# smolGura/fish-tts

Measured on AMD Instinct MI355X. Metric: semantic tokens/sec, higher is better.
Workload: dtype bf16; 1 GPU; openaudio-s1-mini shapes (BASELINE configs[1]): batch=1 per GPU, 48-token prompt, 215 frames (10 s), top-p sampling, hipGraph-captured frame step, + DAC codec decode; prompt_len=48, parallelism=replica x1, frame_engine=3

## Files before the change

fish-tts_amd/csrc/ar_kernels.h:

```cpp
#pragma once
#include "common.h"

namespace ft {

enum { PRO_NONE = 0, PRO_RMSNORM = 1 };
enum { EPI_STORE = 0, EPI_RESID = 1, EPI_SWIGLU = 2 };

__device__ __host__ __forceinline__ size_t xo_index(int m, int k, int ldm) { return ((size_t)(k >> 3) * ldm + m) * 8 + (k & 7); }

struct GemvP {
    const void* W;
    const void* bias;
    const float* x;
    int ldx;
    const void* gain;
    float eps;
    float* out;
    int ldo;
    const float* resid;
    int ldr;
    int N, K;
    int pro, epi;
    int nt;
};
// ... 1396 lines not shown
#pragma unroll
        for (int c = 1; c <= 4; ++c) {
            const unsigned long long bal = __ballot(mine >= c);
            below += __popcll(bal & lower);
            wtot += __popcll(bal);
        }
        if (lane == 0) wcnt[wave] = wtot;
        __syncthreads();
        int rank = below;
        for (int w = 0; w < wave; ++w) rank += wcnt[w];
        bool keep[4];
        float et[4], z2 = 0.f;
#pragma unroll
        for (int e = 0; e < 4; ++e) {
            keep[e] = (i0 + e) < V && (all_kept || key[e] > kstar || (mem[e] && rank < nk));
            rank += mem[e] ? 1 : 0;
            et[e] = keep[e] ? expf(rb<ROUND>(l[e] / Tc) - Mt) : 0.f;
            z2 += et[e];
        }
        const float Z2 = red.sum(z2);
        const float* qrow = nullptr;
        if (p.noise && nfv < p.noise_rows) qrow = p.noise + (size_t)nfv * p.noise_row_len + p.noise_off;
        float q4[4];
        draw_noise4(p, ctl, qrow, i0, nfv, m, V, q4);
        ArgMax best{-1.f, 0x7fffffff};
#pragma unroll
        for (int e = 0; e < 4; ++e) {
            if (i0 + e < V) {
                const float prob = keep[e] ? rb<ROUND>(et[e] / Z2) : 0.f;
                best = better(best, ArgMax{rb<ROUND>(prob / rb<ROUND>(q4[e])), i0 + e});
            }
        }
        winner = block_best(best).i;
    }
    __syncthreads();
    finish_draw<WT>(p, m, winner, nfv);
}

struct SampCut {
    unsigned kstar;
    int nk;
    int all_kept;
    int argmax;
    float Lmax, Mt, Z2, Tc;
};

struct SampBigP {
    SampP s;
    SampCut* cut;
    int* chunk_cnt;
    float* part_score;
    int* part_idx;
    int nchunk;
};

__device__ __forceinline__ float key16_value(unsigned k16) {
    const uint32_t k = k16 << 16;
    const uint32_t u = (k & 0x80000000u) ? (k & 0x7fffffffu) : ~(k | 0xffffu);
    return __uint_as_float(u);
}

constexpr int SAMP_TH_THREADS = 1024;
constexpr int SAMP_TH_ROW = 33;
constexpr int SAMP_TH_OVF = 8;
constexpr size_t SAMP_TH_LDS = (size_t)SAMP_TH_THREADS * SAMP_TH_ROW * 4;

struct SampThShared {
    float red[16];
    int redi[16];
    float wsum[16];
    int wact[16];
    int AL[1024];
    unsigned ovf_key[SAMP_TH_OVF];
    unsigned ovf_cnt[SAMP_TH_OVF];
    int ovf_n;
    SampCut cut_s;
};

__device__ __forceinline__ void samp_cut_from_image(const SampBigP& b, const int m, const uint32_t* cimg, SampThShared& sh,
                                                    const bool has, const int kmax_t) {
    const SampP& p = b.s;
    const int tid = threadIdx.x, lane = tid & 63, wave = tid >> 6;
    const RowCtl ctl = p.ctl[m];
    float* red = sh.red;
    int* redi = sh.redi;
    float* wsum = sh.wsum;
    int* wact = sh.wact;
    int* AL = sh.AL;
    unsigned* ovf_key = sh.ovf_key;
    unsigned* ovf_cnt = sh.ovf_cnt;
    int& ovf_n = sh.ovf_n;
    SampCut& cut_s = sh.cut_s;
    const unsigned long long hb = __ballot(has);
    if (lane == 0) wact[wave] = __popcll(hb);
    __syncthreads();
    int abase = 0, n_active = 0;
    for (int w = 0; w < 16; ++w) { if (w < wave) abase += wact[w]; n_active += wact[w]; }
    if (has) AL[abase + __popcll(hb & ((1ull << lane) - 1ull))] = tid;
    ArgMax km = block_argmax(ArgMax{(float)kmax_t, tid}, red, redi);
    const unsigned kmax = (unsigned)(int)km.v;
    const float Lmax = key16_value(kmax);
    const int n_items = n_active * 64;
    const int ipt = (n_items + 1023) / 1024;
    const int i0 = tid * ipt, i1 = min(i0 + ipt, n_items);
    auto item_count = [&](int i, unsigned& k) -> float {
        const int g = AL[i >> 6], j = i & 63;
        k = 64u * g + j;
        const uint32_t w = cimg[g * SAMP_TH_ROW + (j >> 1)];
        unsigned c = (j & 1) ? (w >> 16) : (w & 0xffffu);
        if (c == 65535u)
            for (int q = 0; q < ovf_n && q < SAMP_TH_OVF; ++q) if (ovf_key[q] == k) c = ovf_cnt[q];
        return (float)c;
    };
    float z = 0.f;
    for (int i = i0; i < i1; ++i) {
        unsigned k;
        const float c = item_count(i, k);
        if (c > 0.f) z = fmaf(c, expf(key16_value(k) - Lmax), z);
    }
    const float Z = block_sum(z, red);
    const float tp = round_bf16(ctl.top_p);
    auto removed = [&](float cum) { return round_bf16(cum) > tp; };
    auto prob = [&](unsigned k16) { return round_bf16(expf(key16_value(k16) - Lmax) / Z); };
    float mt = 0.f;
    for (int i = i0; i < i1; ++i) {
        unsigned k;
        const float c = item_count(i, k);
        if (c > 0.f) mt = fmaf(c, prob(k), mt);
    }
    float suf = mt;
#pragma unroll
    for (int o = 1; o < 64; o <<= 1) {
        const float t = __shfl_down(suf, o, 64);
        if (lane + o < 64) suf += t;
    }
    __syncthreads();
    if (lane == 0) wsum[wave] = suf;
    __syncthreads();
    float above = suf - mt;
    for (int w = wave + 1; w < 16; ++w) above += wsum[w];
    int found = -1;
    unsigned f_key = 0;
    float f_above = 0.f, f_cnt = 0.f;
    float run = above;
    for (int i = i1 - 1; i >= i0; --i) {
        unsigned k;
        const float c = item_count(i, k);
        if (c > 0.f) {
            const float nxt = fmaf(c, prob(k), run);
            if (found < 0 && removed(nxt)) { found = i; f_key = k; f_above = run; f_cnt = c; }
            run = nxt;
        }
    }
    ArgMax who = block_argmax(ArgMax{found >= 0 ? (float)tid : -1.f, tid}, red, redi);
    if (tid == 0) { cut_s.all_kept = who.v < 0.f ? 1 : 0; cut_s.kstar = 0; cut_s.nk = 0; }
    __syncthreads();
    if (who.v >= 0.f && tid == (int)who.v) {
        const float pk = prob(f_key);
        int lo_n = 0, hi_n = (int)f_cnt;
        while (lo_n < hi_n) {
            const int mid = (lo_n + hi_n + 1) >> 1;
            if (removed(fmaf((float)mid, pk, f_above))) hi_n = mid - 1; else lo_n = mid;
        }
        if (f_key == kmax && lo_n < 1) lo_n = 1;
        cut_s.kstar = f_key;
        cut_s.nk = lo_n;
    }
    __syncthreads();
    const unsigned kstar = cut_s.kstar;
    const int nk = cut_s.nk, all_kept = cut_s.all_kept;
    const float Tc = fmaxf(ctl.temperature, 1e-5f);
    const float Mt = round_bf16(Lmax / Tc);
    float z2 = 0.f;
    for (int i = i0; i < i1; ++i) {
        unsigned k;
        const float c = item_count(i, k);
        if (c > 0.f) {
            float n = 0.f;
            if (all_kept || k > kstar) n = c;
            else if (k == kstar) n = (float)nk;
            if (n > 0.f) z2 = fmaf(n, expf(round_bf16(key16_value(k) / Tc) - Mt), z2);
        }
    }
    const float Z2 = block_sum(z2, red);
    if (tid == 0) {
        SampCut o;
        o.kstar = kstar; o.nk = nk; o.all_kept = all_kept; o.argmax = 0;
        o.Lmax = Lmax; o.Mt = Mt; o.Z2 = Z2; o.Tc = Tc;
        b.cut[m] = o;
    }
}

static __global__ __launch_bounds__(1024) void samp_cut_kernel(SampBigP b) {
    extern __shared__ __attribute__((aligned(16))) uint32_t cimg[];
    __shared__ SampThShared sh;
    __shared__ int pen_id[32];
    __shared__ float pen_val[32];
    const SampP& p = b.s;
    const int m = blockIdx.x, tid = threadIdx.x;
    float* L = p.logits + (size_t)m * p.ldl;
    const int V = p.V;
    const RowCtl ctl = p.ctl[m];
    const int nfv = p.nf[m];
    const int R = p.ncb + 1;
    const int* seq = p.seq + (size_t)m * R * p.cap;
    for (int i = tid; i < SAMP_TH_THREADS * SAMP_TH_ROW; i += 1024) cimg[i] = 0u;
    if (tid == 0) sh.ovf_n = 0;
    const int npen = nfv > 0 ? (p.cb == 0 ? R : 16) : 0;
    auto count1 = [&](float v) {
        const unsigned k = order_key(v) >> 16;
        atomicAdd(&cimg[(k >> 6) * SAMP_TH_ROW + ((k & 63u) >> 1)], (k & 1u) ? 0x10000u : 1u);
    };
    {
        if (nfv > 0) {
            const int it = nfv - 1;
            const int ws = it < 16 ? 0 : it - 16;
            if (tid < npen) {
                const int id = p.cb == 0 ? seq[(size_t)tid * p.cap + ws + 1] : seq[(size_t)(p.cb + 1) * p.cap + ws + 1 + tid];
                pen_id[tid] = -1;
                if (id >= 0 && id < V) {
                    const float sv = L[id];
                    pen_id[tid] = id;
                    pen_val[tid] = sv < 0.f ? round_bf16(sv * ctl.rep) : round_bf16(sv / ctl.rep);
                }
            }
            __syncthreads();
            if (tid < npen && pen_id[tid] >= 0) L[pen_id[tid]] = pen_val[tid];
        }
        if (p.cb == 0 && ctl.ban_eos && tid == 0 && p.im_end < V) L[p.im_end] = -INFINITY;
        __syncthreads();
        const int V16 = ((reinterpret_cast<uintptr_t>(L) & 15) == 0) ? (V / 16384) * 16384 : 0;
        float4 fa[4], fb[4];
        auto ld16 = [&](float4 (&f)[4], int base) {
#pragma unroll
            for (int u = 0; u < 4; ++u) f[u] = *reinterpret_cast<const float4*>(L + base + u * 4096 + tid * 4);
        };
        auto cnt16 = [&](const float4 (&f)[4]) {
#pragma unroll
            for (int u = 0; u < 4; ++u) { count1(f[u].x); count1(f[u].y); count1(f[u].z); count1(f[u].w); }
        };
        if (V16 > 0) ld16(fa, 0);
        for (int base = 0; base < V16; base += 32768) {
            if (base + 16384 < V16) ld16(fb, base + 16384);
            cnt16(fa);
            if (base + 32768 < V16) ld16(fa, base + 32768);
            if (base + 16384 < V16) cnt16(fb);
        }
        for (int base = V16; base < V; base += 4096) {
            float f[4];
#pragma unroll
            for (int u = 0; u < 4; ++u) { const int i = base + u * 1024 + tid; f[u] = i < V ? L[i] : 0.f; }
#pragma unroll
            for (int u = 0; u < 4; ++u) if (base + u * 1024 + tid < V) count1(f[u]);
        }
    }
    __syncthreads();
    const uint32_t* row = cimg + tid * SAMP_TH_ROW;
    int kmax_t = -1;
    unsigned tot = 0;
#pragma unroll 8
    for (int j = 0; j < 32; ++j) {
        const uint32_t w = row[j];
        const unsigned c0 = w & 0xffffu, c1 = w >> 16;
        if (c0) kmax_t = 64 * tid + 2 * j;
        if (c1) kmax_t = 64 * tid + 2 * j + 1;
        tot += c0 + c1;
    }
    const int total = (int)block_sum((float)tot, sh.red);
    if (total != V) {
        __shared__ unsigned exc_key[SAMP_TH_OVF];
        __shared__ unsigned exc_cnt[SAMP_TH_OVF];
        for (int i = tid; i < SAMP_TH_THREADS * SAMP_TH_ROW; i += 1024) cimg[i] = 0u;
        if (tid < SAMP_TH_OVF) { exc_key[tid] = 0xffffffffu; exc_cnt[tid] = 0u; }
        __syncthreads();
        for (int i = tid; i < V; i += 1024) {
            const unsigned k = order_key(L[i]) >> 16;
            uint32_t* d = &cimg[(k >> 6) * SAMP_TH_ROW + ((k & 63u) >> 1)];
            const unsigned shft = (k & 1u) * 16u;
            for (;;) {
                const uint32_t old = *reinterpret_cast<volatile uint32_t*>(d);
                if (((old >> shft) & 0xffffu) == 65535u) {
                    for (int q = 0; q < SAMP_TH_OVF; ++q) {
                        const unsigned prev = atomicCAS(&exc_key[q], 0xffffffffu, k);
                        if (prev == 0xffffffffu || prev == k) { atomicAdd(&exc_cnt[q], 1u); break; }
                    }
                    break;
                }
                if (atomicCAS(d, old, old + (1u << shft)) == old) break;
            }
        }
        __syncthreads();
        if (tid == 0) {
            int n = 0;
            for (int q = 0; q < SAMP_TH_OVF; ++q)
                if (exc_key[q] != 0xffffffffu) { sh.ovf_key[n] = exc_key[q]; sh.ovf_cnt[n] = 65535u + exc_cnt[q]; ++n; }
            sh.ovf_n = n;
        }
        kmax_t = -1;
        tot = 0;
        for (int j = 0; j < 32; ++j) {
            const uint32_t w = row[j];
            if (w & 0xffffu) kmax_t = 64 * tid + 2 * j;
            if (w >> 16) kmax_t = 64 * tid + 2 * j + 1;
            tot += (w & 0xffffu) + (w >> 16);
        }
        __syncthreads();
    }
    samp_cut_from_image(b, m, cimg, sh, tot != 0u, kmax_t);
}

static __global__ __launch_bounds__(256) void samp_count_kernel(SampBigP b) {
    __shared__ float red[4];
    const SampP& p = b.s;
    const int m = blockIdx.y, tid = threadIdx.x;
    const int c0 = blockIdx.x * 1024;
    const float* L = p.logits + (size_t)m * p.ldl;
    const SampCut cut = b.cut[m];
    float c = 0.f;
#pragma unroll
    for (int e = 0; e < 4; ++e) {
        const int i = c0 + 4 * tid + e;
        if (i < p.V && (order_key(L[i]) >> 16) == cut.kstar) c += 1.f;
    }
    c = wave_sum(c);
    if ((tid & 63) == 0) red[tid >> 6] = c;
    __syncthreads();
    if (tid == 0) b.chunk_cnt[(size_t)m * b.nchunk + blockIdx.x] = (int)(red[0] + red[1] + red[2] + red[3]);
}

static __global__ __launch_bounds__(256) void samp_race_kernel(SampBigP b) {
    __shared__ float red[4];
    __shared__ int redi[4];
    __shared__ int wcnt[4];
    const SampP& p = b.s;
    const int m = blockIdx.y, tid = threadIdx.x, lane = tid & 63, wave = tid >> 6;
    const int c0 = blockIdx.x * 1024;
    const float* L = p.logits + (size_t)m * p.ldl;
    const int V = p.V;
    const RowCtl ctl = p.ctl[m];
    const int nfv = p.nf[m];
    const SampCut cut = b.cut[m];
    float basef = 0.f;
    for (int i = tid; i < (int)blockIdx.x; i += 256) basef += (float)b.chunk_cnt[(size_t)m * b.nchunk + i];
    basef = wave_sum(basef);
    if (lane == 0) red[wave] = basef;
    __syncthreads();
    const int base = (int)(red[0] + red[1] + red[2] + red[3]);
    __syncthreads();
    float l[4];
    bool member[4];
    int mine = 0;
#pragma unroll
    for (int e = 0; e < 4; ++e) {
        const int i = c0 + 4 * tid + e;
        l[e] = i < V ? L[i] : -INFINITY;
        member[e] = i < V && !cut.all_kept && (order_key(l[e]) >> 16) == cut.kstar;
        mine += member[e] ? 1 : 0;
    }
    int incl = mine;
#pragma unroll
    for (int o = 1; o < 64; o <<= 1) {
// ... 53 lines not shown
```

fish-tts_amd/csrc/engine.h:

```cpp
#pragma once
#include <hip/hip_runtime.h>

#include <map>
#include <string>
#include <vector>

#include "../../include/fishtts_hip.h"
#include "../../include/fishtts_hip_test.h"
#include "common.h"

namespace ft {
struct RowCtl;
struct SampCut;
struct EngLayer;
}

struct FtTensor {
    void* p = nullptr;
    std::vector<int64_t> shape;
    int dtype = FT_BF16;
    int64_t numel() const {
        int64_t n = 1;
        for (auto s : shape) n *= s;
        return n;
// ... 11 lines not shown

struct ft_ctx {
    ft_ar_config c{};
    bool has_ar = false;
    ft_codec_config cc{};
    bool has_codec = false;
    int device = 0;
    hipStream_t stream = nullptr;
    std::string err;
    bool finalized = false;

    std::map<std::string, FtTensor> expected;
    size_t esz = 2;

    void *emb = nullptr, *cb_emb = nullptr, *norm = nullptr, *head = nullptr, *fproj_w = nullptr,
         *fproj_b = nullptr, *fast_emb = nullptr, *fast_norm = nullptr, *fast_out = nullptr;
    float *rope = nullptr, *frope = nullptr;
    std::vector<FtLayer> layers, flayers;

    float *x = nullptr, *qkv = nullptr, *y = nullptr, *g = nullptr, *logits = nullptr, *hid = nullptr,
          *femb = nullptr, *xf = nullptr, *qkvf = nullptr, *gf = nullptr, *flog = nullptr, *part_o = nullptr,
          *part_ml = nullptr;
    int n_slots = 0, nsplit = 1, cap = 0, fastV = 0, y_ld = 0;
    int nsplit_max = 1;
    bool nsplit_fixed = false;
    float *pf_x = nullptr, *pf_qkv = nullptr, *pf_y = nullptr;
    ft::bf16_t *pf_xn = nullptr, *pf_ybf = nullptr, *pf_g = nullptr, *pf_qbf = nullptr;
    int4* pf_seqs = nullptr;
    int2* pf_rows = nullptr;
    ft::bf16_t *xo_x = nullptr, *xo_xf = nullptr, *xo_femb = nullptr, *xo_y = nullptr, *xo_g = nullptr;
    ft::bf16_t* wide_qkv0_tab = nullptr;
    int xo_ldm = 0;
    int xo_pair = 0;
    bool no_attn_wide = false;
    bool no_head_stream = false;
    bool no_pair = false;
    int wide_min = 5;
    bool wide_ok = false;
    bool prefill_v0 = false;
    int prefill_gemm_mode = 2;
    size_t cache_m_stride = 0, fcache_m_stride = 0;

    int *d_pos = nullptr, *d_tok = nullptr, *d_tokn = nullptr, *d_seq = nullptr, *d_nf = nullptr,
        *d_done = nullptr, *d_prompt = nullptr;
    ft::RowCtl* d_ctl = nullptr;
    int *h_pin = nullptr;
    float* noise = nullptr;
    long noise_rows = 0, noise_row_len = 0;

    ft::SampCut* samp_cut = nullptr;
    int* samp_chunk_cnt = nullptr;
    float* samp_part_score = nullptr;
    int* samp_part_idx = nullptr;

    bool eng_on = false;
    bool eng_fast_on = false;
    int eng_nb = 0;
    ft::EngLayer *eng_layers = nullptr, *eng_flayers = nullptr;
    unsigned *eng_gx = nullptr, *eng_gqkv = nullptr, *eng_gy = nullptr, *eng_gxb = nullptr, *eng_gg = nullptr;
    unsigned long long* eng_gpart = nullptr;
    unsigned* eng_fast_g = nullptr;
    unsigned* eng_ctl = nullptr;
    size_t eng_lds_slow = 0, eng_lds_fast = 0, eng_fast_words = 0, eng_pool_words = 0;
    bool eng_relay = true;
    void* eng_qkv0_tab = nullptr;
    bool eng_pair = false;
    bool xl_shape = false;
    bool eng_xl = false;
    std::string path_str;
    const void* eng_slow_fn = nullptr;
    const void* eng_fast_fn = nullptr;
    size_t eng_pool_bytes = 0, eng_gpart_bytes = 0, eng_fast_bytes = 0;
    bool eng_suspended = false;
    int eng_strikes = 0, eng_last_where = 0;
    bool eng_owner = false;
    std::string eng_why;

    std::map<int, hipGraphExec_t> graphs;
    std::map<int, int> graph_nodes;

    bool prof = false, prof_count_only = false;
    std::vector<hipEvent_t> prof_ev;
    int64_t prof_bytes = 0, prof_launches = 0;

    CodecState* codec = nullptr;
};

ft_status ft_fail(ft_ctx* ctx, ft_status code, const std::string& msg);
#define FT_HIP(ctx, call)                                                                         \
    do {                                                                                          \
        hipError_t e_ = (call);                                                                   \
        if (e_ != hipSuccess)                                                                     \
            return ft_fail(ctx, FT_ERR_HIP, std::string(#call) + ": " + hipGetErrorString(e_));  \
    } while (0)

ft_status codec_create(ft_ctx* ctx);
void codec_destroy(ft_ctx* ctx);
void codec_expected(ft_ctx* ctx);
void ft_expect(ft_ctx* ctx, const std::string& name, std::vector<int64_t> shape, int dtype);
ft_status codec_finalize(ft_ctx* ctx);
```

fish-tts_amd/csrc/engine.hip:

```cpp
#include "engine.h"
#include "ar_kernels.h"
#include "frame_engine.h"
#include "wide_kernels.h"
#include "codec_kernels.h"

#include <math.h>

#include <algorithm>
#include <mutex>
#include <stdio.h>
#include <stdlib.h>
#include <string.h>

using namespace ft;

static std::string g_create_err;
static void eng_release(ft_ctx* ctx);

ft_status ft_fail(ft_ctx* ctx, ft_status code, const std::string& msg) {
    if (ctx) ctx->err = msg; else g_create_err = msg;
    return code;
}

template <typename S, typename D>
// ... 138 lines not shown
        FT_TRY(dmalloc(ctx, (char**)&l.vc, M * ctx->cache_m_stride * ctx->esz));
    }
    for (auto& l : ctx->flayers) {
        FT_TRY(dmalloc(ctx, (char**)&l.kc, M * ctx->fcache_m_stride * ctx->esz));
        FT_TRY(dmalloc(ctx, (char**)&l.vc, M * ctx->fcache_m_stride * ctx->esz));
    }
    const size_t R = c.num_codebooks + 1;
    FT_TRY(dmalloc(ctx, &ctx->d_pos, M));
    FT_TRY(dmalloc(ctx, &ctx->d_tok, M * R));
    FT_TRY(dmalloc(ctx, &ctx->d_tokn, M * R));
    FT_TRY(dmalloc(ctx, &ctx->d_seq, M * R * ctx->cap));
    FT_TRY(dmalloc(ctx, &ctx->d_nf, M));
    FT_TRY(dmalloc(ctx, &ctx->d_done, M));
    FT_TRY(dmalloc(ctx, &ctx->d_prompt, R * (size_t)c.max_seq_len));
    FT_TRY(dmalloc(ctx, &ctx->d_ctl, M));
    ctx->prefill_gemm_mode = getenv("FT_PREFILL_GEMM") ? atoi(getenv("FT_PREFILL_GEMM")) : 2;
    ctx->prefill_v0 = getenv("FT_PREFILL_V0") != nullptr || c.dtype != FT_BF16 || c.dim % 32 || (c.n_head * c.head_dim) % 32 ||
                      c.intermediate_size % 32;
    if (!ctx->prefill_v0) {
        const size_t S = c.max_seq_len;
        FT_TRY(dmalloc(ctx, &ctx->pf_x, S * c.dim));
        FT_TRY(dmalloc(ctx, &ctx->pf_qkv, S * qkvN));
        FT_TRY(dmalloc(ctx, &ctx->pf_y, S * c.n_head * c.head_dim));
        FT_TRY(dmalloc(ctx, &ctx->pf_xn, S * c.dim));
        FT_TRY(dmalloc(ctx, &ctx->pf_ybf, S * c.n_head * c.head_dim));
        FT_TRY(dmalloc(ctx, &ctx->pf_g, S * c.intermediate_size));
        FT_TRY(dmalloc(ctx, &ctx->pf_qbf, S * c.n_head * c.head_dim));
        FT_TRY(dmalloc(ctx, &ctx->pf_seqs, M));
        FT_TRY(dmalloc(ctx, &ctx->pf_rows, S));
        const int HD = c.n_head * c.head_dim, HDf = c.fast_n_head * c.fast_head_dim;
        ctx->wide_ok = !getenv("FT_NO_WIDE") && !c.fast_attention_qkv_bias && !c.fast_attention_o_bias && c.fast_dim == c.dim &&
                       wide_k_ok(c.dim) && wide_k_ok(HD) && wide_k_ok(c.intermediate_size) && wide_k_ok(HDf) && wide_k_ok(c.fast_intermediate_size) &&
                       qkvN % 32 == 0 && fqkvN % 32 == 0 && c.intermediate_size % 16 == 0 && c.fast_intermediate_size % 16 == 0 &&
                       c.dim % 16 == 0 && c.vocab_size % 32 == 0 && ctx->fastV % 16 == 0;
        if (ctx->wide_ok) {
            ctx->xo_pair = (int)((M + 15) / 16 * 16);
            ctx->no_pair = getenv("FT_NO_PAIR") != nullptr;
            ctx->no_attn_wide = getenv("FT_NO_ATTN_WIDE") != nullptr;
            ctx->no_head_stream = getenv("FT_NO_HEAD_STREAM") != nullptr;
            ctx->xo_ldm = 2 * ctx->xo_pair;
            const size_t P = ctx->xo_ldm;
            FT_TRY(dmalloc(ctx, &ctx->xo_x, P * c.dim));
            FT_TRY(dmalloc(ctx, &ctx->xo_xf, P * c.fast_dim));
            FT_TRY(dmalloc(ctx, &ctx->xo_femb, P * c.fast_dim));
            FT_TRY(dmalloc(ctx, &ctx->xo_y, P * (size_t)std::max(HD, HDf)));
            FT_TRY(dmalloc(ctx, &ctx->xo_g, P * (size_t)std::max(c.intermediate_size, c.fast_intermediate_size)));
        }
    }
    const size_t nchunk = ((size_t)c.vocab_size + 1023) / 1024;
    FT_TRY(dmalloc(ctx, &ctx->samp_cut, M));
    FT_TRY(dmalloc(ctx, &ctx->samp_chunk_cnt, M * nchunk));
    FT_TRY(dmalloc(ctx, &ctx->samp_part_score, M * nchunk));
    FT_TRY(dmalloc(ctx, &ctx->samp_part_idx, M * nchunk));
    FT_HIP(ctx, hipHostMalloc((void**)&ctx->h_pin, (3 * M + 8) * sizeof(int), hipHostMallocDefault));
    return FT_OK;
}

extern "C" ft_status ft_create(const ft_ar_config* ar, const ft_codec_config* codec, int32_t device, ft_ctx** out) {
    if (!out || (!ar && !codec)) return ft_fail(nullptr, FT_ERR_ARG, "ft_create: need a config and an out pointer");
    int ndev = 0;
    if (hipGetDeviceCount(&ndev) != hipSuccess || ndev == 0)
        return ft_fail(nullptr, FT_ERR_HIP, "ft_create: no HIP device visible (the MI355X path has no CPU fallback)");
    if (device < 0 || device >= ndev) return ft_fail(nullptr, FT_ERR_ARG, "ft_create: bad device index");
    ft_ctx* ctx = new ft_ctx();
    ctx->device = device;
    ft_status st = FT_OK;
    do {
        if (hipSetDevice(device) != hipSuccess) { st = ft_fail(ctx, FT_ERR_HIP, "hipSetDevice failed"); break; }
        if (hipStreamCreateWithFlags(&ctx->stream, hipStreamNonBlocking) != hipSuccess) {
            st = ft_fail(ctx, FT_ERR_HIP, "hipStreamCreate failed"); break;
        }
        if (ar) {
            ctx->c = *ar;
            ctx->has_ar = true;
            if ((st = ar_validate(ctx)) != FT_OK) break;
            if ((st = ar_alloc(ctx)) != FT_OK) break;
            ar_expected(ctx);
        }
        if (codec) {
            ctx->cc = *codec;
            ctx->has_codec = true;
            if ((st = codec_create(ctx)) != FT_OK) break;
            codec_expected(ctx);
        }
    } while (0);
    if (st != FT_OK) {
        g_create_err = ctx->err;
        ft_destroy(ctx);
        return st;
    }
    *out = ctx;
    return FT_OK;
}

extern "C" void ft_destroy(ft_ctx* ctx) {
    if (!ctx) return;
    hipSetDevice(ctx->device);
    if (ctx->stream) hipStreamSynchronize(ctx->stream);
    for (auto& kv : ctx->graphs) hipGraphExecDestroy(kv.second);
    for (auto& kv : ctx->expected) if (kv.second.p) hipFree(kv.second.p);
    for (auto& l : ctx->layers) { hipFree(l.kc); hipFree(l.vc); if (l.w13) hipFree(l.w13); }
    for (auto& l : ctx->flayers) { hipFree(l.kc); hipFree(l.vc); if (l.w13) hipFree(l.w13); }
    float* bufs[] = {ctx->x, ctx->qkv, ctx->y, ctx->g, ctx->logits, ctx->femb, ctx->xf, ctx->qkvf, ctx->gf,
                     ctx->flog, ctx->part_o, ctx->part_ml, ctx->noise};
    for (float* b : bufs) if (b) hipFree(b);
    if (ctx->hid && ctx->hid != ctx->x) hipFree(ctx->hid);
    int* ibufs[] = {ctx->d_pos, ctx->d_tok, ctx->d_tokn, ctx->d_seq, ctx->d_nf, ctx->d_done, ctx->d_prompt};
    for (int* b : ibufs) if (b) hipFree(b);
    if (ctx->d_ctl) hipFree(ctx->d_ctl);
    if (ctx->wide_qkv0_tab) hipFree(ctx->wide_qkv0_tab);
    { void* pf[] = {ctx->pf_x, ctx->pf_qkv, ctx->pf_y, ctx->pf_xn, ctx->pf_ybf, ctx->pf_g, ctx->xo_x, ctx->xo_xf, ctx->xo_femb, ctx->xo_y, ctx->xo_g, ctx->pf_qbf}; for (void* q : pf) if (q) hipFree(q); }
    for (auto& l : ctx->layers) { if (l.bqkv_f32) hipFree(l.bqkv_f32); if (l.bo_f32) hipFree(l.bo_f32); }
    if (ctx->samp_cut) hipFree(ctx->samp_cut);
    if (ctx->samp_chunk_cnt) hipFree(ctx->samp_chunk_cnt);
    if (ctx->samp_part_score) hipFree(ctx->samp_part_score);
    if (ctx->samp_part_idx) hipFree(ctx->samp_part_idx);
    eng_release(ctx);
    if (ctx->h_pin) hipHostFree(ctx->h_pin);
    for (auto e : ctx->prof_ev) hipEventDestroy(e);
    codec_destroy(ctx);
    if (ctx->stream) hipStreamDestroy(ctx->stream);
    delete ctx;
}

extern "C" const char* ft_last_error(const ft_ctx* ctx) { return ctx ? ctx->err.c_str() : g_create_err.c_str(); }

extern "C" ft_status ft_sync(ft_ctx* ctx) {
    if (!ctx) return FT_ERR_ARG;
    FT_HIP(ctx, hipSetDevice(ctx->device));
    FT_HIP(ctx, hipStreamSynchronize(ctx->stream));
    return FT_OK;
}

extern "C" ft_status ft_load_weight(ft_ctx* ctx, const char* name, const void* src, int32_t src_dtype,
                                    const int64_t* shape, int32_t ndim) {
    if (!ctx || !name || !src || !shape) return ft_fail(ctx, FT_ERR_ARG, "ft_load_weight: null argument");
    if (ctx->finalized) return ft_fail(ctx, FT_ERR_STATE, "ft_load_weight: weights already finalized");
    auto it = ctx->expected.find(name);
    if (it == ctx->expected.end()) return ft_fail(ctx, FT_ERR_ARG, std::string("unknown weight name: ") + name);
    FtTensor& t = it->second;
    if ((int)t.shape.size() != ndim) return ft_fail(ctx, FT_ERR_ARG, std::string("rank mismatch for ") + name);
    for (int i = 0; i < ndim; ++i)
        if (t.shape[i] != shape[i]) {
            char buf[256];
            snprintf(buf, sizeof buf, "shape mismatch for %s: dim %d is %lld, expected %lld", name, i,
                     (long long)shape[i], (long long)t.shape[i]);
            return ft_fail(ctx, FT_ERR_ARG, buf);
        }
    if (src_dtype != FT_F32 && src_dtype != FT_BF16 && src_dtype != FT_F16)
        return ft_fail(ctx, FT_ERR_ARG, "src_dtype must be FT_F32, FT_BF16 or FT_F16");
    FT_HIP(ctx, hipSetDevice(ctx->device));
    const int64_t n = t.numel();
    const size_t ssz = src_dtype == FT_F32 ? 4 : 2, dsz = t.dtype == FT_F32 ? 4 : 2;
    if (!t.p) FT_HIP(ctx, hipMalloc(&t.p, (size_t)n * dsz + 64));
    if (src_dtype == t.dtype) {
        FT_HIP(ctx, hipMemcpy(t.p, src, (size_t)n * dsz, hipMemcpyDefault));
        return FT_OK;
    }
    void* stage = nullptr;
    FT_HIP(ctx, hipMalloc(&stage, (size_t)n * ssz));
    hipError_t e = hipMemcpy(stage, src, (size_t)n * ssz, hipMemcpyDefault);
    if (e == hipSuccess) {
        const int blocks = (int)((n + 255) / 256 < 4096 ? (n + 255) / 256 : 4096);
        auto to = [&](auto* sp) {
            if (t.dtype == FT_F32) convert_kernel<<<blocks, 256, 0, ctx->stream>>>(sp, (float*)t.p, n);
            else if (t.dtype == FT_BF16) convert_kernel<<<blocks, 256, 0, ctx->stream>>>(sp, (bf16_t*)t.p, n);
            else convert_kernel<<<blocks, 256, 0, ctx->stream>>>(sp, (f16_t*)t.p, n);
        };
        if (src_dtype == FT_F32) to((const float*)stage);
// ... 727 lines not shown
                                                                             ctx->xo_x + (size_t)L.m0 * 8, ctx->xo_ldm);
            L.chk();
        }
        if constexpr (ROUND == RND_BF16)
            wide_gemm(L, ctx->xo_x + (size_t)L.m0 * 8, ctx->head, nullptr, c.vocab_size, c.dim, ctx->norm, WEPI_STORE,
                      ctx->logits + (size_t)L.m0 * c.vocab_size, c.vocab_size, nullptr, nullptr, 0, true);
        return;
    }
    GemvP h{};
    h.W = ctx->head; h.x = ctx->x + (size_t)L.m0 * c.dim; h.ldx = c.dim; h.gain = ctx->norm; h.eps = c.norm_eps;
    h.out = ctx->logits + (size_t)L.m0 * c.vocab_size; h.ldo = c.vocab_size; h.N = c.vocab_size; h.K = c.dim;
    h.pro = PRO_RMSNORM; h.epi = EPI_STORE; h.nt = 1;
    gemv<WT, ROUND>(L, h, rows_per_wave(h.N, L.M));
}

template <typename WT, int ROUND>
static void enqueue_sample(Launch& L, int cb, bool last) {
    if (L.gemv_only) return;
    ft_ctx* ctx = L.ctx;
    const ft_ar_config& c = ctx->c;
    const int m0 = L.m0, R = c.num_codebooks + 1;
    SampP s{};
    if (cb == 0) { s.logits = ctx->logits + (size_t)m0 * c.vocab_size; s.ldl = c.vocab_size; s.V = c.vocab_size; }
    else { s.logits = ctx->flog + (size_t)m0 * ctx->fastV; s.ldl = ctx->fastV; s.V = ctx->fastV; }
    s.ctl = ctx->d_ctl + m0; s.tokn = ctx->d_tokn + (size_t)m0 * R; s.seq = ctx->d_seq + (size_t)m0 * R * ctx->cap;
    s.cap = ctx->cap; s.nf = ctx->d_nf + m0; s.cb = cb; s.ncb = c.num_codebooks; s.sem_begin = c.semantic_begin_id;
    s.im_end = c.im_end_id; s.cbsize = c.codebook_size; s.fast_emb = ctx->fast_emb;
    s.femb = ctx->femb + (size_t)m0 * c.fast_dim; s.Df = c.fast_dim; s.noise = ctx->noise;
    s.noise_row_len = ctx->noise_row_len; s.noise_rows = ctx->noise_rows;
    s.noise_off = cb == 0 ? 0 : (long)c.vocab_size + (long)(cb - 1) * ctx->fastV;
    s.last = last ? 1 : 0; s.tok = ctx->d_tok + (size_t)m0 * R; s.pos = ctx->d_pos + m0; s.done = ctx->d_done + m0;
    if (wide_batch(L)) {
        s.femb_xo = (cb == 0 && wide_pair(L) ? ctx->xo_x + (size_t)ctx->xo_pair * 8 : ctx->xo_femb) + (size_t)m0 * 8;
        s.femb_ldm = ctx->xo_ldm;
        if (cb >= 1 && cb + 1 < c.num_codebooks && ctx->wide_qkv0_tab) {
            s.qkv0_tab = ctx->wide_qkv0_tab; s.qkv0_n = (c.fast_n_head + 2 * c.fast_n_local_heads) * c.fast_head_dim;
            s.qkv0_out = ctx->qkvf + (size_t)m0 * s.qkv0_n;
        }
    }
    if (s.V <= 1024) {
        sample_small_kernel<WT, ROUND><<<L.M, 256, 0, L.s>>>(s);
    } else if (ROUND == RND_BF16) {
        SampBigP b{};
        b.s = s; b.nchunk = (s.V + 1023) / 1024;
        b.cut = ctx->samp_cut + m0;
        b.chunk_cnt = ctx->samp_chunk_cnt + (size_t)m0 * b.nchunk;
        b.part_score = ctx->samp_part_score + (size_t)m0 * b.nchunk;
        b.part_idx = ctx->samp_part_idx + (size_t)m0 * b.nchunk;
        const dim3 gridc(b.nchunk, L.M);
        {
            static DevOnce once;
            once.run([] {
                hipFuncSetAttribute((const void*)samp_cut_kernel, hipFuncAttributeMaxDynamicSharedMemorySize, (int)SAMP_TH_LDS);
            });
        }
        samp_cut_kernel<<<L.M, SAMP_TH_THREADS, SAMP_TH_LDS, L.s>>>(b);
        samp_count_kernel<<<gridc, 256, 0, L.s>>>(b);
        samp_race_kernel<<<gridc, 256, 0, L.s>>>(b);
        samp_finish_kernel<WT><<<L.M, 256, 0, L.s>>>(b);
    } else {
        sample_block_kernel<WT, ROUND><<<L.M, 1024, 0, L.s>>>(s);
    }
    L.chk();
}

template <typename WT, int ROUND>
static void enqueue_fast_step(Launch& L, const int cb, const bool pair = false) {
    ft_ctx* ctx = L.ctx;
    const ft_ar_config& c = ctx->c;
    const int m0 = L.m0;
    const int Df = c.fast_dim, Hf = c.fast_n_head, Hkvf = c.fast_n_local_heads, hdf = c.fast_head_dim;
    const size_t qkvN = (size_t)(Hf + 2 * Hkvf) * hdf;
    float* xf = ctx->xf + (size_t)m0 * Df;
    float* qkvf = ctx->qkvf + (size_t)m0 * qkvN;
    float* gf = ctx->gf + (size_t)m0 * c.fast_intermediate_size;
    {
        const float* xin = cb == 0 ? ctx->hid + (size_t)m0 * Df : ctx->femb + (size_t)m0 * Df;
        const bool wide = wide_batch(L);
        for (int li = 0; li < c.n_fast_layer; ++li) {
            const FtLayer& l = ctx->flayers[li];
            const float* xl = li == 0 ? xin : xf;
            if (wide) {
                if constexpr (ROUND == RND_BF16) {
                    const int HDf = Hf * hdf, Ff = c.fast_intermediate_size, M = L.M, ldm = ctx->xo_ldm;
                    const int rows = pair ? ctx->xo_pair + M : M;
                    const bf16_t* xin_o = ((cb == 0 || pair) ? ctx->xo_x : ctx->xo_femb) + (size_t)m0 * 8;
                    bf16_t* xfo = ctx->xo_xf + (size_t)m0 * 8;
                    bf16_t* yo = ctx->xo_y + (size_t)m0 * 8;
                    bf16_t* go = ctx->xo_g + (size_t)m0 * 8;
                    const bf16_t* xlo = li == 0 ? xin_o : xfo;
                    if (!(li == 0 && cb >= 2 && !pair && ctx->wide_qkv0_tab))
                        wide_gemm(L, xlo, l.wqkv, nullptr, (int)qkvN, Df, l.attn_norm, WEPI_STORE, qkvf, (long)qkvN, nullptr, nullptr, rows);
                    FastAttnP a{};
                    a.qkv = qkvf; a.ldq = (int)qkvN; a.qn = l.qn; a.kn = l.kn; a.rope = ctx->frope;
                    a.kc = (char*)l.kc + (size_t)m0 * ctx->fcache_m_stride * ctx->esz;
                    a.vc = (char*)l.vc + (size_t)m0 * ctx->fcache_m_stride * ctx->esz;
                    a.cache_m_stride = ctx->fcache_m_stride; a.c = pair ? 0 : cb; a.H = Hf; a.Hkv = Hkvf; a.hd = hdf;
                    a.ncb = c.num_codebooks; a.eps = c.norm_eps; a.scale = (float)(1.0 / sqrt((double)hdf));
                    a.y_bf = yo; a.y_xo_ldm = ldm;
                    a.pair_M = pair ? M : 0; a.pair_off = ctx->xo_pair;
                    fast_attn_kernel<WT, ROUND><<<dim3(Hf, pair ? 2 * M : M), 64, 0, L.s>>>(a, nullptr, HDf);
                    L.chk();
                    wide_gemm(L, yo, l.wo, nullptr, Df, HDf, nullptr, WEPI_RESID, nullptr, 0, xfo, xlo, rows);
                    wide_gemm(L, xfo, l.w13, nullptr, 2 * Ff, Df, l.ffn_norm, WEPI_SWIGLU, nullptr, 0, go, nullptr, rows);
                    wide_gemm(L, go, l.w2, nullptr, Df, Ff, nullptr, WEPI_RESID, nullptr, 0, xfo, xfo, rows);
                }
                continue;
            }
            GemvP p{};
// ... 914 lines not shown
```

Measured before the change: 780.8 tokens/s.

## Split top-p cut histogram across multiple blocks with last-block merge

After: 784.6 tokens/s, median of 6. Within noise of the previous version (+0.5%).

```diff
diff --git a/fish-tts_amd/csrc/ar_kernels.h b/fish-tts_amd/csrc/ar_kernels.h
--- a/fish-tts_amd/csrc/ar_kernels.h
+++ b/fish-tts_amd/csrc/ar_kernels.h
@@ -1472,7 +1472,21 @@
     float* part_score;
     int* part_idx;
     int nchunk;
+    uint32_t* pub;
+    unsigned long long* pub_bm;
+    unsigned* arrive;
+    int nb;
 };
+
+#ifdef FT_SAMP_STAMPS
+__device__ unsigned long long* samp_stamps;
+#define SAMP_STAMP(k) do { __syncthreads(); \
+    if (threadIdx.x == 0 && samp_stamps) samp_stamps[((size_t)blockIdx.y * gridDim.x + blockIdx.x) * 16 + (k)] = __builtin_amdgcn_s_memrealtime(); } while (0)
+#define SAMP_NOTE(k, v) do { if (threadIdx.x == 0 && samp_stamps) samp_stamps[((size_t)blockIdx.y * gridDim.x + blockIdx.x) * 16 + (k)] = (v); } while (0)
+#else
+#define SAMP_STAMP(k) do {} while (0)
+#define SAMP_NOTE(k, v) do {} while (0)
+#endif
 
 __device__ __forceinline__ float key16_value(unsigned k16) {
     const uint32_t k = k16 << 16;
@@ -1484,6 +1498,15 @@
 constexpr int SAMP_TH_ROW = 33;
 constexpr int SAMP_TH_OVF = 8;
 constexpr size_t SAMP_TH_LDS = (size_t)SAMP_TH_THREADS * SAMP_TH_ROW * 4;
+constexpr int SAMP_CACHE = 8;
+constexpr int SAMP_SPLIT_NB = 16;
+inline int samp_split_nb(int V, int M, int cus) {
+    int n = (V + 8191) / 8192;
+    n = n > SAMP_SPLIT_NB ? SAMP_SPLIT_NB : n;
+    const int fit = cus / (M > 0 ? M : 1);
+    n = n > fit ? (fit < 2 ? 2 : fit) : n;
+    return n < 1 ? 1 : n > SAMP_SPLIT_NB ? SAMP_SPLIT_NB : n;
+}
 
 struct SampThShared {
     float red[16];
@@ -1491,38 +1514,34 @@
     float wsum[16];
     int wact[16];
     int AL[1024];
+    unsigned long long bmw[SAMP_SPLIT_NB * 16];
     unsigned ovf_key[SAMP_TH_OVF];
     unsigned ovf_cnt[SAMP_TH_OVF];
     int ovf_n;
     SampCut cut_s;
 };
 
-__device__ __forceinline__ void samp_cut_from_image(const SampBigP& b, const int m, const uint32_t* cimg, SampThShared& sh,
-                                                    const bool has, const int kmax_t) {
+template <int CACHE>
+__device__ __forceinline__ void samp_cut_search(const SampBigP& b, const int m, const uint32_t* cimg, SampThShared& sh,
+                                                const unsigned kmax, const int n_items) {
     const SampP& p = b.s;
     const int tid = threadIdx.x, lane = tid & 63, wave = tid >> 6;
     const RowCtl ctl = p.ctl[m];
     float* red = sh.red;
     int* redi = sh.redi;
     float* wsum = sh.wsum;
-    int* wact = sh.wact;
-    int* AL = sh.AL;
-    unsigned* ovf_key = sh.ovf_key;
-    unsigned* ovf_cnt = sh.ovf_cnt;
-    int& ovf_n = sh.ovf_n;
+    const int* AL = sh.AL;
+    const unsigned* ovf_key = sh.ovf_key;
+    const unsigned* ovf_cnt = sh.ovf_cnt;
+    const int ovf_n = sh.ovf_n;
     SampCut& cut_s = sh.cut_s;
-    const unsigned long long hb = __ballot(has);
-    if (lane == 0) wact[wave] = __popcll(hb);
-    __syncthreads();
-    int abase = 0, n_active = 0;
-    for (int w = 0; w < 16; ++w) { if (w < wave) abase += wact[w]; n_active += wact[w]; }
-    if (has) AL[abase + __popcll(hb & ((1ull << lane) - 1ull))] = tid;
-    ArgMax km = block_argmax(ArgMax{(float)kmax_t, tid}, red, redi);
-    const unsigned kmax = (unsigned)(int)km.v;
     const float Lmax = key16_value(kmax);
-    const int n_items = n_active * 64;
     const int ipt = (n_items + 1023) / 1024;
     const int i0 = tid * ipt, i1 = min(i0 + ipt, n_items);
+    const int n = i1 > i0 ? i1 - i0 : 0;
+    constexpr int NU = CACHE > 0 ? CACHE : 1;
+    unsigned ck[NU];
+    float cc[NU], ce[NU], cp[NU];
     auto item_count = [&](int i, unsigned& k) -> float {
         const int g = AL[i >> 6], j = i & 63;
         k = 64u * g + j;
@@ -1532,21 +1551,38 @@
             for (int q = 0; q < ovf_n && q < SAMP_TH_OVF; ++q) if (ovf_key[q] == k) c = ovf_cnt[q];
         return (float)c;
     };
+    auto item = [&](int u, unsigned& k) -> float {
+        if constexpr (CACHE > 0) { k = ck[u]; return cc[u]; }
+        else return item_count(i0 + u, k);
+    };
     float z = 0.f;
-    for (int i = i0; i < i1; ++i) {
+#pragma unroll
+    for (int u = 0; u < (CACHE > 0 ? CACHE : n); ++u) {
+        if (CACHE > 0 && u >= n) break;
         unsigned k;
-        const float c = item_count(i, k);
-        if (c > 0.f) z = fmaf(c, expf(key16_value(k) - Lmax), z);
+        const float c = item_count(i0 + u, k);
+        const float e = c > 0.f ? expf(key16_value(k) - Lmax) : 0.f;
+        if constexpr (CACHE > 0) { ck[u] = k; cc[u] = c; ce[u] = e; }
+        if (c > 0.f) z = fmaf(c, e, z);
     }
     const float Z = block_sum(z, red);
+    SAMP_STAMP(5);
     const float tp = round_bf16(ctl.top_p);
     auto removed = [&](float cum) { return round_bf16(cum) > tp; };
     auto prob = [&](unsigned k16) { return round_bf16(expf(key16_value(k16) - Lmax) / Z); };
     float mt = 0.f;
-    for (int i = i0; i < i1; ++i) {
+#pragma unroll
+    for (int u = 0; u < (CACHE > 0 ? CACHE : n); ++u) {
+        if (CACHE > 0 && u >= n) break;
         unsigned k;
-        const float c = item_count(i, k);
-        if (c > 0.f) mt = fmaf(c, prob(k), mt);
+        const float c = item(u, k);
+        float pr = 0.f;
+        if (c > 0.f) {
+            if constexpr (CACHE > 0) pr = round_bf16(ce[u] / Z);
+            else pr = prob(k);
+            mt = fmaf(c, pr, mt);
+        }
+        if constexpr (CACHE > 0) cp[u] = pr;
     }
     float suf = mt;
 #pragma unroll
@@ -1559,20 +1595,27 @@
     __syncthreads();
     float above = suf - mt;
     for (int w = wave + 1; w < 16; ++w) above += wsum[w];
-    int found = -1;
+    SAMP_STAMP(6);
+    bool found = false;
     unsigned f_key = 0;
     float f_above = 0.f, f_cnt = 0.f;
     float run = above;
-    for (int i = i1 - 1; i >= i0; --i) {
+#pragma unroll
+    for (int u = (CACHE > 0 ? CACHE : n) - 1; u >= 0; --u) {
+        if (CACHE > 0 && u >= n) continue;
         unsigned k;
-        const float c = item_count(i, k);
+        const float c = item(u, k);
         if (c > 0.f) {
-            const float nxt = fmaf(c, prob(k), run);
-            if (found < 0 && removed(nxt)) { found = i; f_key = k; f_above = run; f_cnt = c; }
+            float pr;
+            if constexpr (CACHE > 0) pr = cp[u];
+            else pr = prob(k);
+            const float nxt = fmaf(c, pr, run);
+            if (!found && removed(nxt)) { found = true; f_key = k; f_above = run; f_cnt = c; }
             run = nxt;
         }
     }
-    ArgMax who = block_argmax(ArgMax{found >= 0 ? (float)tid : -1.f, tid}, red, redi);
+    ArgMax who = block_argmax(ArgMax{found ? (float)tid : -1.f, tid}, red, redi);
+    SAMP_STAMP(7);
     if (tid == 0) { cut_s.all_kept = who.v < 0.f ? 1 : 0; cut_s.kstar = 0; cut_s.nk = 0; }
     __syncthreads();
     if (who.v >= 0.f && tid == (int)who.v) {
@@ -1587,28 +1630,95 @@
         cut_s.nk = lo_n;
     }
     __syncthreads();
+    SAMP_STAMP(8);
     const unsigned kstar = cut_s.kstar;
     const int nk = cut_s.nk, all_kept = cut_s.all_kept;
     const float Tc = fmaxf(ctl.temperature, 1e-5f);
     const float Mt = round_bf16(Lmax / Tc);
     float z2 = 0.f;
-    for (int i = i0; i < i1; ++i) {
+#pragma unroll
+    for (int u = 0; u < (CACHE > 0 ? CACHE : n); ++u) {
+        if (CACHE > 0 && u >= n) break;
         unsigned k;
-        const float c = item_count(i, k);
+        const float c = item(u, k);
         if (c > 0.f) {
-            float n = 0.f;
-            if (all_kept || k > kstar) n = c;
-            else if (k == kstar) n = (float)nk;
-            if (n > 0.f) z2 = fmaf(n, expf(round_bf16(key16_value(k) / Tc) - Mt), z2);
+            float nn = 0.f;
+            if (all_kept || k > kstar) nn = c;
+            else if (k == kstar) nn = (float)nk;
+            if (nn > 0.f) z2 = fmaf(nn, expf(round_bf16(key16_value(k) / Tc) - Mt), z2);
         }
     }
     const float Z2 = block_sum(z2, red);
+    SAMP_STAMP(9);
     if (tid == 0) {
         SampCut o;
         o.kstar = kstar; o.nk = nk; o.all_kept = all_kept; o.argmax = 0;
         o.Lmax = Lmax; o.Mt = Mt; o.Z2 = Z2; o.Tc = Tc;
         b.cut[m] = o;
     }
+}
+
+__device__ __forceinline__ void samp_cut_from_image(const SampBigP& b, const int m, const uint32_t* cimg, SampThShared& sh,
+                                                    const bool has, const int kmax_t) {
+    const int tid = threadIdx.x, lane = tid & 63, wave = tid >> 6;
+    const unsigned long long hb = __ballot(has);
+    if (lane == 0) sh.wact[wave] = __popcll(hb);
+    __syncthreads();
+    int abase = 0, n_active = 0;
+    for (int w = 0; w < 16; ++w) { if (w < wave) abase += sh.wact[w]; n_active += sh.wact[w]; }
+    if (has) sh.AL[abase + __popcll(hb & ((1ull << lane) - 1ull))] = tid;
+    ArgMax km = block_argmax(ArgMax{(float)kmax_t, tid}, sh.red, sh.redi);
+    SAMP_STAMP(4);
+    const unsigned kmax = (unsigned)(int)km.v;
+    const int n_items = n_active * 64;
+    if (n_items <= SAMP_CACHE * 1024) samp_cut_search<SAMP_CACHE>(b, m, cimg, sh, kmax, n_items);
+    else samp_cut_search<0>(b, m, cimg, sh, kmax, n_items);
+}
+
+template <bool SC1>
+__device__ void samp_recount_exact(const float* L, const int V, uint32_t* cimg, SampThShared& sh, int& kmax_t, unsigned& tot) {
+    const int tid = threadIdx.x;
+    __shared__ unsigned exc_key[SAMP_TH_OVF];
+    __shared__ unsigned exc_cnt[SAMP_TH_OVF];
+    __syncthreads();
+    for (int i = tid; i < SAMP_TH_THREADS * SAMP_TH_ROW; i += 1024) cimg[i] = 0u;
+    if (tid < SAMP_TH_OVF) { exc_key[tid] = 0xffffffffu; exc_cnt[tid] = 0u; }
+    __syncthreads();
+    for (int i = tid; i < V; i += 1024) {
+        const float v = SC1 ? __uint_as_float(__hip_atomic_load(reinterpret_cast<const uint32_t*>(L) + i, __ATOMIC_RELAXED,
+                                                                 __HIP_MEMORY_SCOPE_AGENT)) : L[i];
+        const unsigned k = order_key(v) >> 16;
+        uint32_t* d = &cimg[(k >> 6) * SAMP_TH_ROW + ((k & 63u) >> 1)];
+        const unsigned shft = (k & 1u) * 16u;
+        for (;;) {
+            const uint32_t old = *reinterpret_cast<volatile uint32_t*>(d);
+            if (((old >> shft) & 0xffffu) == 65535u) {
+                for (int q = 0; q < SAMP_TH_OVF; ++q) {
+                    const unsigned prev = atomicCAS(&exc_key[q], 0xffffffffu, k);
+                    if (prev == 0xffffffffu || prev == k) { atomicAdd(&exc_cnt[q], 1u); break; }
+                }
+                break;
+            }
+            if (atomicCAS(d, old, old + (1u << shft)) == old) break;
+        }
+    }
+    __syncthreads();
+    if (tid == 0) {
+        int n = 0;
+        for (int q = 0; q < SAMP_TH_OVF; ++q)
+            if (exc_key[q] != 0xffffffffu) { sh.ovf_key[n] = exc_key[q]; sh.ovf_cnt[n] = 65535u + exc_cnt[q]; ++n; }
+        sh.ovf_n = n;
+    }
+    const uint32_t* row = cimg + tid * SAMP_TH_ROW;
+    kmax_t = -1;
+    tot = 0;
+    for (int j = 0; j < 32; ++j) {
+        const uint32_t w = row[j];
+        if (w & 0xffffu) kmax_t = 64 * tid + 2 * j;
+        if (w >> 16) kmax_t = 64 * tid + 2 * j + 1;
+        tot += (w & 0xffffu) + (w >> 16);
+    }
+    __syncthreads();
 }
 
 static __global__ __launch_bounds__(1024) void samp_cut_kernel(SampBigP b) {
@@ -1624,8 +1734,10 @@
     const int nfv = p.nf[m];
     const int R = p.ncb + 1;
     const int* seq = p.seq + (size_t)m * R * p.cap;
+    SAMP_STAMP(0);
     for (int i = tid; i < SAMP_TH_THREADS * SAMP_TH_ROW; i += 1024) cimg[i] = 0u;
     if (tid == 0) sh.ovf_n = 0;
+    SAMP_STAMP(1);
     const int npen = nfv > 0 ? (p.cb == 0 ? R : 16) : 0;
     auto count1 = [&](float v) {
         const unsigned k = order_key(v) >> 16;
@@ -1675,6 +1787,7 @@
         }
     }
     __syncthreads();
+    SAMP_STAMP(2);
     const uint32_t* row = cimg + tid * SAMP_TH_ROW;
     int kmax_t = -1;
     unsigned tot = 0;
@@ -1687,46 +1800,152 @@
         tot += c0 + c1;
     }
     const int total = (int)block_sum((float)tot, sh.red);
+    if (total != V) samp_recount_exact<false>(L, V, cimg, sh, kmax_t, tot);
+    SAMP_STAMP(3);
+    samp_cut_from_image(b, m, cimg, sh, tot != 0u, kmax_t);
+}
+
+static __global__ __launch_bounds__(1024) void samp_split_kernel(SampBigP b) {
+    extern __shared__ __attribute__((aligned(16))) uint32_t cimg[];
+    __shared__ SampThShared sh;
+    __shared__ int pen_id[32];
+    __shared__ float pen_val[32];
+    __shared__ int last_s;
+    const SampP& p = b.s;
+    const int j = blockIdx.x, m = blockIdx.y, tid = threadIdx.x, lane = tid & 63, wave = tid >> 6;
+    const int nb = b.nb;
+    float* L = p.logits + (size_t)m * p.ldl;
+    const int V = p.V;
+    const int S = (((V + nb - 1) / nb) + 1023) & ~1023;
+    const int lo = min(j * S, V), hi = min(lo + S, V);
+    const RowCtl ctl = p.ctl[m];
+    const int nfv = p.nf[m];
+    const int R = p.ncb + 1;
+    const int* seq = p.seq + (size_t)m * R * p.cap;
+    SAMP_STAMP(0);
+    for (int i = tid; i < SAMP_TH_THREADS * SAMP_TH_ROW; i += 1024) cimg[i] = 0u;
+    if (tid == 0) sh.ovf_n = 0;
+    SAMP_STAMP(1);
+    const int npen = nfv > 0 ? (p.cb == 0 ? R : 16) : 0;
+    if (nfv > 0) {
+        const int it = nfv - 1;
+        const int ws = it < 16 ? 0 : it - 16;
+        if (tid < npen) {
+            const int id = p.cb == 0 ? seq[(size_t)tid * p.cap + ws + 1] : seq[(size_t)(p.cb + 1) * p.cap + ws + 1 + tid];
+            pen_id[tid] = -1;
+            if (id >= lo && id < hi) {
+                const float sv = L[id];
+                pen_id[tid] = id;
+                pen_val[tid] = sv < 0.f ? round_bf16(sv * ctl.rep) : round_bf16(sv / ctl.rep);
+            }
+        }
+        __syncthreads();
+        if (tid < npen && pen_id[tid] >= 0) L[pen_id[tid]] = pen_val[tid];
+    }
+    const bool ban = p.cb == 0 && ctl.ban_eos && p.im_end >= lo && p.im_end < hi;
+    if (ban && tid == 0) L[p.im_end] = -INFINITY;
+    __syncthreads();
+    auto count1 = [&](float v) {
+        const unsigned k = order_key(v) >> 16;
+        atomicAdd(&cimg[(k >> 6) * SAMP_TH_ROW + ((k & 63u) >> 1)], (k & 1u) ? 0x10000u : 1u);
+    };
+    for (int base = lo; base < hi; base += 4096) {
+        float f[4];
+#pragma unroll
+        for (int u = 0; u < 4; ++u) { const int i = base + u * 1024 + tid; f[u] = i < hi ? L[i] : 0.f; }
+#pragma unroll
+        for (int u = 0; u < 4; ++u) if (base + u * 1024 + tid < hi) count1(f[u]);
+    }
+    __syncthreads();
+    SAMP_STAMP(2);
+    const uint32_t* row = cimg + tid * SAMP_TH_ROW;
+    uint32_t w32[32];
+    bool mine = false;
+#pragma unroll
+    for (int q = 0; q < 32; ++q) { w32[q] = row[q]; mine |= w32[q] != 0u; }
+    const unsigned long long hb = __ballot(mine);
+    const size_t slot = (size_t)m * nb + j;
+    if (mine) {
+        unsigned long long* dst = reinterpret_cast<unsigned long long*>(b.pub + (slot * 1024 + tid) * 32);
+#pragma unroll
+        for (int q = 0; q < 16; ++q)
+            __hip_atomic_store(dst + q, (unsigned long long)w32[2 * q] | ((unsigned long long)w32[2 * q + 1] << 32), __ATOMIC_RELAXED,
+                               __HIP_MEMORY_SCOPE_AGENT);
+    }
+    if (lane == 0) __hip_atomic_store(b.pub_bm + slot * 16 + wave, hb, __ATOMIC_RELAXED, __HIP_MEMORY_SCOPE_AGENT);
+    if (nfv > 0 && tid < npen && pen_id[tid] >= 0)
+        __hip_atomic_store(reinterpret_cast<uint32_t*>(L) + pen_id[tid], __float_as_uint(pen_val[tid]), __ATOMIC_RELAXED,
+                           __HIP_MEMORY_SCOPE_AGENT);
+    if (ban && tid == 0)
+        __hip_atomic_store(reinterpret_cast<uint32_t*>(L) + p.im_end, __float_as_uint(-INFINITY), __ATOMIC_RELAXED,
+                           __HIP_MEMORY_SCOPE_AGENT);
+    asm volatile("s_waitcnt vmcnt(0)" ::: "memory");
+    __syncthreads();
+    if (tid == 0) {
+        const unsigned prev = __hip_atomic_fetch_add(b.arrive + m, 1u, __ATOMIC_RELAXED, __HIP_MEMORY_SCOPE_AGENT);
+        const int last = prev == (unsigned)(nb - 1);
+        if (last) __hip_atomic_store(b.arrive + m, 0u, __ATOMIC_RELAXED, __HIP_MEMORY_SCOPE_AGENT);
+        last_s = last;
+    }
+    __syncthreads();
+    if (!last_s) return;
+    unsigned long long bm[SAMP_SPLIT_NB];
+#pragma unroll
+    for (int o = 0; o < SAMP_SPLIT_NB; ++o)
+        bm[o] = o >= nb ? 0ull : o == j ? hb : __hip_atomic_load(b.pub_bm + ((size_t)m * nb + o) * 16 + wave, __ATOMIC_RELAXED,
+                                                                __HIP_MEMORY_SCOPE_AGENT);
+    unsigned long long un = 0ull;
+#pragma unroll
+    for (int o = 0; o < SAMP_SPLIT_NB; ++o) {
+        un |= bm[o];
+        if (lane == o) sh.bmw[o * 16 + wave] = bm[o];
+    }
+    const bool occ = (un >> lane) & 1ull;
+    if (lane == 0) sh.wact[wave] = __popcll(un);
+    __syncthreads();
+    int abase = 0, n_occ = 0;
+    for (int w = 0; w < 16; ++w) { if (w < wave) abase += sh.wact[w]; n_occ += sh.wact[w]; }
+    if (occ) sh.AL[abase + __popcll(un & ((1ull << lane) - 1ull))] = tid;
+    __syncthreads();
+    int kmax_t = -1;
+    unsigned tot = 0;
+    const int q = tid & 7;
+    for (int gi = tid >> 3; gi < n_occ; gi += 128) {
+        const int g = sh.AL[gi];
+        unsigned long long v0[SAMP_SPLIT_NB], v1[SAMP_SPLIT_NB];
+#pragma unroll
+        for (int o = 0; o < SAMP_SPLIT_NB; ++o) {
+            v0[o] = 0ull; v1[o] = 0ull;
+            if (o < nb && o != j && ((sh.bmw[o * 16 + (g >> 6)] >> (g & 63)) & 1ull)) {
+                const unsigned long long* src =
+                    reinterpret_cast<const unsigned long long*>(b.pub + (((size_t)m * nb + o) * 1024 + g) * 32 + 4 * q);
+                v0[o] = __hip_atomic_load(src, __ATOMIC_RELAXED, __HIP_MEMORY_SCOPE_AGENT);
+                v1[o] = __hip_atomic_load(src + 1, __ATOMIC_RELAXED, __HIP_MEMORY_SCOPE_AGENT);
+            }
+        }
+        uint32_t* dst = cimg + g * SAMP_TH_ROW + 4 * q;
+        U4 w{dst[0], dst[1], dst[2], dst[3]};
+#pragma unroll
+        for (int o = 0; o < SAMP_SPLIT_NB; ++o)
+            w += U4{(uint32_t)v0[o], (uint32_t)(v0[o] >> 32), (uint32_t)v1[o], (uint32_t)(v1[o] >> 32)};
+#pragma unroll
+        for (int e = 0; e < 4; ++e) {
+            dst[e] = w[e];
+            const unsigned c0 = w[e] & 0xffffu, c1 = w[e] >> 16;
+            if (c0) kmax_t = max(kmax_t, 64 * g + 8 * q + 2 * e);
+            if (c1) kmax_t = max(kmax_t, 64 * g + 8 * q + 2 * e + 1);
+            tot += c0 + c1;
+        }
+    }
+    const int total = (int)block_sum((float)tot, sh.red);
+    bool has = occ;
+    SAMP_NOTE(10, (unsigned long long)total); SAMP_NOTE(11, (unsigned long long)n_occ);
     if (total != V) {
-        __shared__ unsigned exc_key[SAMP_TH_OVF];
-        __shared__ unsigned exc_cnt[SAMP_TH_OVF];
-        for (int i = tid; i < SAMP_TH_THREADS * SAMP_TH_ROW; i += 1024) cimg[i] = 0u;
-        if (tid < SAMP_TH_OVF) { exc_key[tid] = 0xffffffffu; exc_cnt[tid] = 0u; }
-        __syncthreads();
-        for (int i = tid; i < V; i += 1024) {
-            const unsigned k = order_key(L[i]) >> 16;
-            uint32_t* d = &cimg[(k >> 6) * SAMP_TH_ROW + ((k & 63u) >> 1)];
-            const unsigned shft = (k & 1u) * 16u;
-            for (;;) {
-                const uint32_t old = *reinterpret_cast<volatile uint32_t*>(d);
-                if (((old >> shft) & 0xffffu) == 65535u) {
-                    for (int q = 0; q < SAMP_TH_OVF; ++q) {
-                        const unsigned prev = atomicCAS(&exc_key[q], 0xffffffffu, k);
-                        if (prev == 0xffffffffu || prev == k) { atomicAdd(&exc_cnt[q], 1u); break; }
-                    }
-                    break;
-                }
-                if (atomicCAS(d, old, old + (1u << shft)) == old) break;
-            }
-        }
-        __syncthreads();
-        if (tid == 0) {
-            int n = 0;
-            for (int q = 0; q < SAMP_TH_OVF; ++q)
-                if (exc_key[q] != 0xffffffffu) { sh.ovf_key[n] = exc_key[q]; sh.ovf_cnt[n] = 65535u + exc_cnt[q]; ++n; }
-            sh.ovf_n = n;
-        }
-        kmax_t = -1;
-        tot = 0;
-        for (int j = 0; j < 32; ++j) {
-            const uint32_t w = row[j];
-            if (w & 0xffffu) kmax_t = 64 * tid + 2 * j;
-            if (w >> 16) kmax_t = 64 * tid + 2 * j + 1;
-            tot += (w & 0xffffu) + (w >> 16);
-        }
-        __syncthreads();
-    }
-    samp_cut_from_image(b, m, cimg, sh, tot != 0u, kmax_t);
+        samp_recount_exact<true>(L, V, cimg, sh, kmax_t, tot);
+        has = tot != 0u;
+    }
+    SAMP_STAMP(3);
+    samp_cut_from_image(b, m, cimg, sh, has, kmax_t);
 }
 
 static __global__ __launch_bounds__(256) void samp_count_kernel(SampBigP b) {
diff --git a/fish-tts_amd/csrc/engine.h b/fish-tts_amd/csrc/engine.h
--- a/fish-tts_amd/csrc/engine.h
+++ b/fish-tts_amd/csrc/engine.h
@@ -87,6 +87,11 @@
     int* samp_chunk_cnt = nullptr;
     float* samp_part_score = nullptr;
     int* samp_part_idx = nullptr;
+    bool samp_split = false;
+    uint32_t* samp_pub = nullptr;
+    unsigned long long* samp_pub_bm = nullptr;
+    unsigned* samp_arrive = nullptr;
+    int samp_cus = 256;
 
     bool eng_on = false;
     bool eng_fast_on = false;
diff --git a/fish-tts_amd/csrc/engine.hip b/fish-tts_amd/csrc/engine.hip
--- a/fish-tts_amd/csrc/engine.hip
+++ b/fish-tts_amd/csrc/engine.hip
@@ -214,6 +214,14 @@
     FT_TRY(dmalloc(ctx, &ctx->samp_chunk_cnt, M * nchunk));
     FT_TRY(dmalloc(ctx, &ctx->samp_part_score, M * nchunk));
     FT_TRY(dmalloc(ctx, &ctx->samp_part_idx, M * nchunk));
+    ctx->samp_split = c.dtype == FT_BF16 && c.vocab_size > 1024 && !getenv("FT_NO_SAMP_SPLIT");
+    if (ctx->samp_split) {
+        FT_TRY(dmalloc(ctx, &ctx->samp_pub, M * SAMP_SPLIT_NB * 1024 * 32));
+        FT_TRY(dmalloc(ctx, &ctx->samp_pub_bm, M * SAMP_SPLIT_NB * 16));
+        FT_TRY(dmalloc(ctx, &ctx->samp_arrive, M));
+        hipDeviceProp_t prop;
+        if (hipGetDeviceProperties(&prop, ctx->device) == hipSuccess && prop.multiProcessorCount > 0) ctx->samp_cus = prop.multiProcessorCount;
+    }
     FT_HIP(ctx, hipHostMalloc((void**)&ctx->h_pin, (3 * M + 8) * sizeof(int), hipHostMallocDefault));
     return FT_OK;
 }
@@ -277,6 +285,9 @@
     if (ctx->samp_chunk_cnt) hipFree(ctx->samp_chunk_cnt);
     if (ctx->samp_part_score) hipFree(ctx->samp_part_score);
     if (ctx->samp_part_idx) hipFree(ctx->samp_part_idx);
+    if (ctx->samp_pub) hipFree(ctx->samp_pub);
+    if (ctx->samp_pub_bm) hipFree(ctx->samp_pub_bm);
+    if (ctx->samp_arrive) hipFree(ctx->samp_arrive);
     eng_release(ctx);
     if (ctx->h_pin) hipHostFree(ctx->h_pin);
     for (auto e : ctx->prof_ev) hipEventDestroy(e);
@@ -1110,9 +1121,18 @@
             static DevOnce once;
             once.run([] {
                 hipFuncSetAttribute((const void*)samp_cut_kernel, hipFuncAttributeMaxDynamicSharedMemorySize, (int)SAMP_TH_LDS);
+                hipFuncSetAttribute((const void*)samp_split_kernel, hipFuncAttributeMaxDynamicSharedMemorySize, (int)SAMP_TH_LDS);
             });
         }
-        samp_cut_kernel<<<L.M, SAMP_TH_THREADS, SAMP_TH_LDS, L.s>>>(b);
+        if (ctx->samp_split) {
+            b.nb = samp_split_nb(s.V, L.M, ctx->samp_cus);
+            b.pub = ctx->samp_pub + (size_t)m0 * SAMP_SPLIT_NB * 1024 * 32;
+            b.pub_bm = ctx->samp_pub_bm + (size_t)m0 * SAMP_SPLIT_NB * 16;
+            b.arrive = ctx->samp_arrive + m0;
+            samp_split_kernel<<<dim3(b.nb, L.M), SAMP_TH_THREADS, SAMP_TH_LDS, L.s>>>(b);
+        } else {
+            samp_cut_kernel<<<L.M, SAMP_TH_THREADS, SAMP_TH_LDS, L.s>>>(b);
+        }
         samp_count_kernel<<<gridc, 256, 0, L.s>>>(b);
         samp_race_kernel<<<gridc, 256, 0, L.s>>>(b);
         samp_finish_kernel<WT><<<L.M, 256, 0, L.s>>>(b);
```
